# snphbaum/scikit-gpuppy

Measured on NVIDIA B200. Metric: fit_s_per_iter, lower is better.
Workload: dtype f64

## Files before the change

### scikit-gpuppy_b200/csrc/gpk.cu

```cuda
#include "../../include/gpk.h"
#include "../../include/gpk_test.h"

#include <climits>
#include <new>
#include <vector>

#include "dgemm_dmma.cuh"
#include "factor.cuh"
#include "se_kernels.cuh"
#include "exact_kernels.cuh"
#include "periodic_kernels.cuh"

namespace gpk {
thread_local char g_err[512] = {0};
thread_local long g_launch_count = 0;
thread_local bool g_prof_on = false;
static thread_local std::vector<ProfPair> g_prof;
void prof_push(cudaEvent_t a, cudaEvent_t b) { g_prof.push_back(ProfPair{a, b}); }

struct Handle {
  int n = 0, d = 0, npad = 0;
  double *X = nullptr, *W = nullptr;
  bool own_X = false, own_W = false;
  double *x = nullptr, *xT = nullptr, *t = nullptr, *y = nullptr, *alpha = nullptr, *dL = nullptr;
// ... 1088 lines not shown
  op.sl = reinterpret_cast<int8_t*>(planes_out); op.sc = scales_out;
  op.rows = (int)rows; op.K = (int)K; op.S = moduli;
  unsigned long long* mx = nullptr;
  GPK_CUDA_OK(cudaMalloc((void**)&mx, (size_t)rows * sizeof(unsigned long long)));
  int rc = oz::slice_operand(src, ld, trans, lower, op, mx, st);
  cudaError_t e = cudaStreamSynchronize(st);
  cudaFree(mx);
  if (rc < 0) return rc;
  if (e != cudaSuccess) { snprintf(g_err, sizeof(g_err), "oz_residues: %s", cudaGetErrorString(e)); return -1; }
  return 0;
}

int gpk_test_oz_gemm(const double* A, int64_t lda, int transA, int lowerA, const double* B, int64_t ldb, int transB,
                     int lowerB, double* C, int64_t ldc, int64_t M, int64_t N, int64_t K, double alpha, double beta,
                     int krange, int lower_only, int moduli, int64_t panel_rows, int reps, float* ms_out, void* stream) {
  cudaStream_t st = reinterpret_cast<cudaStream_t>(stream);
  oz::Operand a, b;
  a.rows = (int)M; a.K = (int)K; a.S = moduli;
  b.rows = (int)N; b.K = (int)K; b.S = moduli;
  unsigned long long* mx = nullptr;
  cudaEvent_t e0 = nullptr, e1 = nullptr, e2 = nullptr;
  int rc = 0;
  auto cleanup = [&]() {
    cudaFree(a.sl); cudaFree(a.sc); cudaFree(b.sl); cudaFree(b.sc); cudaFree(mx); cudaFree(a.out);
    if (e0) cudaEventDestroy(e0);
    if (e1) cudaEventDestroy(e1);
    if (e2) cudaEventDestroy(e2);
  };
#define OZ_OK(expr)                                                                         \
  do {                                                                                      \
    cudaError_t _e = (expr);                                                                \
    if (_e != cudaSuccess) {                                                                \
      snprintf(g_err, sizeof(g_err), "oz_gemm: %s -> %s", #expr, cudaGetErrorString(_e));   \
      cleanup();                                                                            \
      return -1;                                                                            \
    }                                                                                       \
  } while (0)
  OZ_OK(cudaMalloc((void**)&a.sl, oz::Operand::slice_bytes(a.rows, a.K, a.S)));
  OZ_OK(cudaMalloc((void**)&b.sl, oz::Operand::slice_bytes(b.rows, b.K, b.S)));
  OZ_OK(cudaMalloc((void**)&a.sc, (size_t)M * sizeof(double)));
  OZ_OK(cudaMalloc((void**)&b.sc, (size_t)N * sizeof(double)));
  OZ_OK(cudaMalloc((void**)&mx, (size_t)(M > N ? M : N) * sizeof(unsigned long long)));
  {
    const long prow = panel_rows > 0 ? round_up_l((long)panel_rows, 256) : round_up_l((long)M, 256);
    size_t want_out = (size_t)a.S * prow * round_up_l((long)N, 256);
    if (want_out > ((size_t)16 << 30)) want_out = (size_t)16 << 30;
    OZ_OK(cudaMalloc((void**)&a.out, want_out));
    a.out_cap = want_out;
  }
  OZ_OK(cudaEventCreate(&e0));
  OZ_OK(cudaEventCreate(&e1));
  OZ_OK(cudaEventCreate(&e2));
  OZ_OK(cudaEventRecord(e0, st));
  rc = oz::slice_operand(A, lda, transA, lowerA, a, mx, st);
  if (rc == 0) rc = oz::slice_operand(B, ldb, transB, lowerB, b, mx, st);
  if (rc < 0) { cleanup(); return rc; }
  OZ_OK(cudaEventRecord(e1, st));
  if (reps < 1) reps = 1;
  for (int r = 0; r < reps && rc == 0; ++r) rc = oz::gemm_sliced(a, b, C, ldc, alpha, beta, krange, lower_only, st);
  if (rc < 0) { cleanup(); return rc; }
  OZ_OK(cudaEventRecord(e2, st));
  OZ_OK(cudaStreamSynchronize(st));
  if (ms_out) {
    OZ_OK(cudaEventElapsedTime(&ms_out[0], e0, e1));
    OZ_OK(cudaEventElapsedTime(&ms_out[1], e1, e2));
    ms_out[1] /= reps;
  }
#undef OZ_OK
  cleanup();
  return 0;
}

int gpk_test_tune(int group_m, int recon_cw) {
  if (group_m > 0) oz::g_group_m = group_m;
  if (recon_cw == 1 || recon_cw == 2 || recon_cw == 4) oz::g_recon_cw = recon_cw;
  return 0;
}

int gpk_test_position_lock(int on) {
  if (on >= 0 && on <= 2) oz::g_position_lock = on;
  return oz::g_position_lock;
}

int gpk_test_overlap(int on) {
  if (on == 0 || on == 1) g_overlap_T = on;
  return g_overlap_T;
}

int gpk_profile(int on) {
  g_prof_on = on != 0;
  return 0;
}

int gpk_profile_read(double* gemm_ms, int64_t* gemm_launches, int64_t* all_launches, double* max_gemm_ms) {
  double total = 0.0, longest = 0.0;
  for (auto& p : g_prof) {
    float ms = 0.f;
    cudaError_t e = cudaEventSynchronize(p.b);
    if (e == cudaSuccess) e = cudaEventElapsedTime(&ms, p.a, p.b);
    cudaEventDestroy(p.a);
    cudaEventDestroy(p.b);
    if (e != cudaSuccess) {
      snprintf(g_err, sizeof(g_err), "gpk_profile_read: %s", cudaGetErrorString(e));
      g_prof.clear();
      return -1;
    }
    total += ms;
    if (ms > longest) longest = ms;
  }
  if (max_gemm_ms) *max_gemm_ms = longest;
  if (gemm_ms) *gemm_ms = total;
  if (gemm_launches) *gemm_launches = (int64_t)g_prof.size();
  if (all_launches) *all_launches = (int64_t)g_launch_count;
  g_prof.clear();
  g_launch_count = 0;
  return 0;
}

int gpk_microbench_i8(int64_t iters, double seconds, double* out_host) {
  int nsm = 0, dev = 0;
  GPK_CUDA_OK(cudaGetDevice(&dev));
  GPK_CUDA_OK(cudaDeviceGetAttribute(&nsm, cudaDevAttrMultiProcessorCount, dev));
  const int smem = 2 * oz::TILE_BYTES + 1024 + 64;
  GPK_CUDA_OK(cudaFuncSetAttribute(mb_i8_kernel, cudaFuncAttributeMaxDynamicSharedMemorySize, smem));
  cudaLaunchConfig_t cfg;
  memset(&cfg, 0, sizeof(cfg));
  cudaLaunchAttribute attr[1];
  attr[0].id = cudaLaunchAttributeClusterDimension;
  attr[0].val.clusterDim.x = 2;
  attr[0].val.clusterDim.y = 1;
  attr[0].val.clusterDim.z = 1;
  const int pairs = nsm / 2;
  cfg.gridDim = dim3(2 * pairs);
  cfg.blockDim = dim3(128);
  cfg.dynamicSmemBytes = smem;
  cfg.stream = nullptr;
  cfg.attrs = attr;
  cfg.numAttrs = 1;
  cudaEvent_t e0, e1;
  GPK_CUDA_OK(cudaEventCreate(&e0));
  GPK_CUDA_OK(cudaEventCreate(&e1));
  const double ops_per_launch = (double)pairs * (double)iters * 4.0 * 256.0 * 256.0 * 32.0 * 2.0;
  long it = iters;
  double best = 0.0;
  for (int rep = 0; rep < 4; ++rep) {
    GPK_CUDA_OK(cudaEventRecord(e0));
    GPK_CUDA_OK(cudaLaunchKernelEx(&cfg, mb_i8_kernel, it));
    GPK_LAUNCH_OK();
    GPK_CUDA_OK(cudaEventRecord(e1));
    GPK_CUDA_OK(cudaEventSynchronize(e1));
    float ms = 0.f;
    GPK_CUDA_OK(cudaEventElapsedTime(&ms, e0, e1));
    const double tops = ops_per_launch / (ms * 1e-3) / 1e12;
    if (rep > 0 && tops > best) best = tops;
  }
  out_host[0] = best;
  out_host[1] = 0.0;
  if (seconds > 0.0) {
    const double per_launch_s = ops_per_launch / (best * 1e12);
    long launches = (long)(seconds / per_launch_s) + 1;
    GPK_CUDA_OK(cudaEventRecord(e0));
    for (long l = 0; l < launches; ++l) {
      GPK_CUDA_OK(cudaLaunchKernelEx(&cfg, mb_i8_kernel, it));
      GPK_LAUNCH_OK();
    }
    GPK_CUDA_OK(cudaEventRecord(e1));
// ... 36 lines not shown
```

### scikit-gpuppy_b200/csrc/oz_crt_planes.cuh

```cuda

struct PlaneArgs {
  uint8_t* res; long res_ld; long res_plane;
  int M, N, K;
  int row_tile0;
  int krange, lower_only, group_m;
  int widen, band_cols;
  int nmod;
  unsigned int* phase;
  int* spill;
  int m[CRT_MAX_MODULI]; uint32_t magic[CRT_MAX_MODULI]; uint32_t u[CRT_MAX_MODULI];
};

constexpr int RECON_GROUPS = (CRT_MAX_MODULI + 3) / 4;

struct ReconArgs {
  const uint8_t* res; long res_ld; long res_plane;
  double* C; long ldc;
  const double* scA; const double* scB;
  double alpha, beta;
  int M, N, K;
  int row0;
  long ncols_pad;
  int krange, lower_only;
  int nmod;
  double p_scaled;
  double* colsq; double* pairdot; long ldo;
  uint32_t wp[2 * RECON_GROUPS][6];
};

constexpr int SPILL_SLOTS = 256;
constexpr int Q_BN = 256;
constexpr int Q_STAGES = 7;
constexpr int Q_STAGE_BYTES = 2 * TILE_BYTES;
constexpr int Q_SMEM_BYTES = Q_STAGES * Q_STAGE_BYTES + 1024 + 256;

__host__ __device__ __forceinline__ void planes_krange(int krange, int K, int bi2, int bx2, int& kb0, int& kb1) {
  kb0 = 0;
  kb1 = K / BK;
  switch (krange) {
    case K_UPTO_BJ: kb1 = (kb1 < 2 * bx2 + 2) ? kb1 : 2 * bx2 + 2; break;
    case K_FROM_BJ: kb0 = (kb1 < 2 * bx2) ? kb1 : 2 * bx2; break;
    case K_UPTO_BI: kb1 = (kb1 < 2 * bi2 + 2) ? kb1 : 2 * bi2 + 2; break;
    case K_FROM_BI: kb0 = (kb1 < 2 * bi2) ? kb1 : 2 * bi2; break;
    default: break;
  }
}

__global__ void __launch_bounds__(THREADS, 1)
oz_crt_planes_kernel(const __grid_constant__ CUtensorMap tmA, const __grid_constant__ CUtensorMap tmB,
                     const __grid_constant__ PlaneArgs p) {
  extern __shared__ uint8_t oz_smem_raw[];
  const int warp = threadIdx.x >> 5, lane = threadIdx.x & 31;
  const uint32_t rank = cluster_ctarank();
  const int pp = (int)(rank & 1u);

  int bx = blockIdx.x >> 1, by = blockIdx.y;
  const int nx = gridDim.x >> 1, ny = (int)gridDim.y;
  int band_lo = 0, band_hi = 0;
  if (p.group_m > 0) {
    const int pid = by * nx + bx;
    if (!p.band_cols) {
      const int per_band = p.group_m * nx;
      const int band = pid / per_band;
      const int first = band * p.group_m;
      const int rows = min(ny - first, p.group_m);
      const int rem = pid - band * per_band;
      by = first + rem % rows;
      bx = rem / rows;
      band_lo = first + p.row_tile0;
      band_hi = first + rows - 1 + p.row_tile0;
    } else {
      const int per_band = p.group_m * ny;
      const int band = pid / per_band;
      const int first = band * p.group_m;
      const int cols = min(nx - first, p.group_m);
      const int rem = pid - band * per_band;
      bx = first + rem % cols;
      by = rem / cols;
      band_lo = first;
      band_hi = first + cols - 1;
    }
  }
  const int bi2 = by + p.row_tile0;
  const int bi = 2 * bi2 + pp;
  const int bjt = 2 * bx + pp;
  if (p.lower_only && 2 * bx > 2 * bi2 + 1) return;
  int kb0, kb1;
  planes_krange(p.krange, p.K, bi2, bx, kb0, kb1);
  if (kb1 <= kb0) return;
  if (p.widen) {
    const int kbt = p.K / BK;
    switch (p.krange) {
      case K_FROM_BI: case K_FROM_BJ: { const int u = min(kb0, 2 * band_lo); kb0 = max(u, kb0 - WIDEN_TILES); if (kb0 < 0) kb0 = 0; } break;
      case K_UPTO_BI: case K_UPTO_BJ: { const int u = max(kb1, min(kbt, 2 * band_hi + 2)); kb1 = min(u, kb1 + WIDEN_TILES); if (kb1 > kbt) kb1 = kbt; } break;
      default: break;
    }
  }
  const int nmod = p.nmod;

  const uint32_t raw = smem_u32(oz_smem_raw);
  uint8_t* smem = oz_smem_raw + ((1024u - (raw & 1023u)) & 1023u);
  uint64_t* bars = reinterpret_cast<uint64_t*>(smem + Q_STAGES * Q_STAGE_BYTES);
  uint64_t* full = bars;
  uint64_t* empty = bars + Q_STAGES;
  uint64_t* tmem_full = bars + 2 * Q_STAGES;
  uint64_t* tmem_empty = bars + 2 * Q_STAGES + 2;
  uint32_t* tmem_slot = reinterpret_cast<uint32_t*>(bars + 2 * Q_STAGES + 4);

  if (warp == 0 && lane == 0) {
    tma_prefetch_desc(&tmA);
    tma_prefetch_desc(&tmB);
  }
  if (warp == 1 && lane == 0) {
    for (int s = 0; s < Q_STAGES; ++s) {
      mbar_init(&full[s], 1);
      mbar_init(&empty[s], 1);
    }
    for (int b = 0; b < 2; ++b) {
      mbar_init(&tmem_full[b], 1);
      mbar_init(&tmem_empty[b], 2 * EPI_WARPS);
    }
    fence_barrier_init();
  }
  if (warp == 2) tmem_alloc_pair(tmem_slot, TMEM_COLS);
  uint32_t* phase_slot = tmem_slot + 1;
  if (rank == 0 && threadIdx.x == 0) *phase_slot = p.phase ? *reinterpret_cast<volatile unsigned int*>(p.phase) : 0u;
  tc_fence_before();
  cluster_sync_all();
  tc_fence_after();
  const uint32_t tmem_base = *tmem_slot;
  uint32_t phase0;
  asm volatile(
      "{\n\t.reg .b32 ra;\n\t"
      "mapa.shared::cluster.u32 ra, %1, 0;\n\t"
      "ld.shared::cluster.u32 %0, [ra];\n\t}\n"
      : "=r"(phase0)
      : "r"(smem_u32(phase_slot))
      : "memory");
  uint32_t smid;
  asm volatile("mov.u32 %0, %%smid;" : "=r"(smid));
  const int nk = kb1 - kb0;
  uint32_t mstep0 = phase0 >> 16;
  int k_start = kb0 + (int)(phase0 & 0xffffu);
  if (k_start >= kb1) { k_start = kb0; ++mstep0; }
  const bool split = k_start > kb0 && p.spill != nullptr;
  if (!split) k_start = kb0;
  const int i0 = (int)(mstep0 % (uint32_t)nmod);
  const int nseg = nmod + (split ? 1 : 0);
#define SEG_MOD(sx) ((sx) < nmod ? ((i0 + (sx)) >= nmod ? i0 + (sx) - nmod : i0 + (sx)) : i0)
#define SEG_BEG(sx) ((split && (sx) == 0) ? k_start : kb0)
#define SEG_END(sx) ((split && (sx) == nmod) ? k_start : kb1)

  if (warp == 0) {
    if (lane == 0) {
      int stage = 0;
      uint32_t phase = 0;
      for (int sg = 0; sg < nseg; ++sg) {
        const int i = SEG_MOD(sg);
        const int kbeg = SEG_BEG(sg), kend = SEG_END(sg);
        for (int kb = kbeg; kb < kend; ++kb) {
          if (rank == 0 && p.phase && sg < nmod && ((kb - kbeg) & 3) == 0)
            atomicMax(p.phase, ((mstep0 + (uint32_t)sg) << 16) | (uint32_t)(kb - kb0));
          mbar_wait(&empty[stage], phase ^ 1u);
          uint8_t* st = smem + stage * Q_STAGE_BYTES;
          if (pp == 0) mbar_expect_tx(&full[stage], 2u * (uint32_t)Q_STAGE_BYTES);
          tma_load_tile_pair(st, &tmA, &full[stage], 0, kb, bi, i);
          tma_load_tile_pair(st + TILE_BYTES, &tmB, &full[stage], 0, kb, bjt, i);
          if (++stage == Q_STAGES) { stage = 0; phase ^= 1u; }
        }
      }
    }
  } else if (warp == 1) {
    if (lane == 0 && pp == 0) {
      constexpr uint32_t idesc = umma_idesc_i8(2 * BM, Q_BN);
      int stage = 0;
      uint32_t phase = 0;
      for (int sg = 0; sg < nseg; ++sg) {
        const int buf = sg & 1;
        if (sg >= 2) {
          mbar_wait(&tmem_empty[buf], (uint32_t)((sg >> 1) - 1) & 1u);
          tc_fence_after();
        }
        const uint32_t acc = tmem_base + (uint32_t)(buf * Q_BN);
        const int kbeg = SEG_BEG(sg), kend = SEG_END(sg);
        for (int kb = kbeg; kb < kend; ++kb) {
          mbar_wait(&full[stage], phase);
          tc_fence_after();
          const uint32_t st = smem_u32(smem + stage * Q_STAGE_BYTES);
          const uint64_t ad = umma_desc_sw128(st);
          const uint64_t bd = umma_desc_sw128(st + TILE_BYTES);
#pragma unroll
          for (int k4 = 0; k4 < BK / 32; ++k4)
            umma_i8_pair(acc, ad + (uint64_t)(k4 * 2), bd + (uint64_t)(k4 * 2), idesc, (kb > kbeg) | (k4 > 0));
          umma_commit_pair(&empty[stage], 3);
          if (++stage == Q_STAGES) { stage = 0; phase ^= 1u; }
        }
        umma_commit_pair(&tmem_full[buf], 3);
      }
    }
  } else {
    const int quad = warp & 3, half = (warp - 2) >> 2;
    const int row = quad * 32 + lane;
    const uint32_t lane_addr = tmem_base + ((uint32_t)(quad * 32) << 16);
    const long lrow = (long)by * (2 * BM) + pp * BM + row;
    uint8_t* dst0 = p.res + lrow * p.res_ld + (long)bx * Q_BN + half * 128;
    int4* sp = split ? reinterpret_cast<int4*>(p.spill + ((size_t)(smid % SPILL_SLOTS) * BM + row) * Q_BN + half * 128) : nullptr;
    for (int sg = 0; sg < nseg; ++sg) {
      const int i = SEG_MOD(sg);
      const bool spill_out = split && sg == 0, add_in = split && sg == nmod;
      const int buf = sg & 1;
      if (lane == 0) mbar_wait(&tmem_full[buf], (uint32_t)(sg >> 1) & 1u);
      __syncwarp();
      tc_fence_after();
      const int m = p.m[i];
      const int magic = (int)p.magic[i];
      const uint32_t u = p.u[i];
      uint8_t* dst = dst0 + (long)i * p.res_plane;
#pragma unroll
      for (int c = 0; c < 4; ++c) {
        uint32_t R[2][16];
        const uint32_t ta = lane_addr + (uint32_t)(buf * Q_BN + half * 128 + c * 32);
        tmem_ld16(ta, R[0]);
        tmem_ld16(ta + 16u, R[1]);
        tmem_ld_wait();
        if (c == 3) {
          tc_fence_before();
          __syncwarp();
          if (lane == 0) mbar_arrive_cluster(&tmem_empty[buf], rank & ~1u);
        }
        if (spill_out) {
#pragma unroll
          for (int x = 0; x < 8; ++x) {
            const uint32_t* r4 = &R[x >> 2][(x & 3) * 4];
            sp[c * 8 + x] = make_int4((int)r4[0], (int)r4[1], (int)r4[2], (int)r4[3]);
          }
          continue;
        }
        if (add_in) {
#pragma unroll
          for (int x = 0; x < 8; ++x) {
            const int4 v = sp[c * 8 + x];
            uint32_t* r4 = &R[x >> 2][(x & 3) * 4];
            r4[0] += (uint32_t)v.x; r4[1] += (uint32_t)v.y; r4[2] += (uint32_t)v.z; r4[3] += (uint32_t)v.w;
          }
        }
        uint32_t pk[8];
#pragma unroll
        for (int x = 0; x < 32; ++x) {
          const int Rv = (int)R[x >> 4][x & 15];
          const int r = Rv - __mulhi(Rv, magic) * m + m;
          const uint32_t t = (uint32_t)r * u;
          uint32_t s = t - __umulhi(t, (uint32_t)magic) * (uint32_t)m;
          s = (s >= (uint32_t)m) ? s - (uint32_t)m : s;
          if ((x & 3) == 0) pk[x >> 2] = s;
          else pk[x >> 2] |= s << (8 * (x & 3));
        }
        uint4* o = reinterpret_cast<uint4*>(dst + c * 32);
        o[0] = make_uint4(pk[0], pk[1], pk[2], pk[3]);
        o[1] = make_uint4(pk[4], pk[5], pk[6], pk[7]);
      }
    }
  }
#undef SEG_MOD
#undef SEG_BEG
#undef SEG_END
  tc_fence_before();
  cluster_sync_all();
  if (warp == 2) tmem_dealloc_pair(tmem_base, TMEM_COLS);
}

__device__ __forceinline__ uint32_t dp2a_lo(uint32_t a, uint32_t b, uint32_t c) {
  uint32_t d;
  asm("dp2a.lo.u32.u32 %0, %1, %2, %3;" : "=r"(d) : "r"(a), "r"(b), "r"(c));
  return d;
}
__device__ __forceinline__ uint32_t dp2a_hi(uint32_t a, uint32_t b, uint32_t c) {
  uint32_t d;
  asm("dp2a.hi.u32.u32 %0, %1, %2, %3;" : "=r"(d) : "r"(a), "r"(b), "r"(c));
  return d;
}
// ... 103 lines not shown
```

### scikit-gpuppy_b200/csrc/oz_gemm.cuh

```cuda
#pragma once
#include <cuda.h>

#include "dgemm_dmma.cuh"
#include "oz_crt_tables.h"

namespace gpk {
namespace oz {

constexpr int BM = 128, BN = 128, BK = 128;
constexpr int TILE_BYTES = BM * BK;
constexpr int EPI_WARPS = 8;
constexpr int THREADS = 64 + EPI_WARPS * 32;
constexpr int TMEM_COLS = 512;

constexpr int OZ_EPI_STORE = 0;
constexpr int OZ_EPI_ROWSQ = 1;

__device__ __forceinline__ uint32_t smem_u32(const void* p) { return (uint32_t)__cvta_generic_to_shared(p); }

__device__ __forceinline__ void mbar_init(uint64_t* bar, uint32_t count) {
  asm volatile("mbarrier.init.shared::cta.b64 [%0], %1;" ::"r"(smem_u32(bar)), "r"(count) : "memory");
}
__device__ __forceinline__ void fence_barrier_init() {
  asm volatile("fence.mbarrier_init.release.cluster;" ::: "memory");
}
__device__ __forceinline__ void mbar_expect_tx(uint64_t* bar, uint32_t bytes) {
  asm volatile("mbarrier.arrive.expect_tx.shared::cta.b64 _, [%0], %1;" ::"r"(smem_u32(bar)), "r"(bytes) : "memory");
}
__device__ __forceinline__ void mbar_arrive(uint64_t* bar) {
  asm volatile("mbarrier.arrive.shared::cta.b64 _, [%0];" ::"r"(smem_u32(bar)) : "memory");
}
__device__ __forceinline__ bool mbar_try_wait(uint64_t* bar, uint32_t parity) {
  uint32_t ok;
  asm volatile(
      "{\n\t.reg .pred p;\n\t"
      "mbarrier.try_wait.parity.shared::cta.b64 p, [%1], %2;\n\t"
      "selp.u32 %0, 1, 0, p;\n\t}\n"
      : "=r"(ok)
      : "r"(smem_u32(bar)), "r"(parity)
      : "memory");
  return ok != 0;
}
__device__ __forceinline__ void mbar_wait(uint64_t* bar, uint32_t parity) {
  if (mbar_try_wait(bar, parity)) return;
  const long long t0 = clock64();
  while (!mbar_try_wait(bar, parity)) {
    if (clock64() - t0 > 4000000000LL) __trap();
  }
}
__device__ __forceinline__ void tma_prefetch_desc(const CUtensorMap* tm) {
  asm volatile("prefetch.tensormap [%0];" ::"l"(tm) : "memory");
}
__device__ __forceinline__ void tc_fence_before() { asm volatile("tcgen05.fence::before_thread_sync;" ::: "memory"); }
__device__ __forceinline__ void tc_fence_after() { asm volatile("tcgen05.fence::after_thread_sync;" ::: "memory"); }
__device__ __forceinline__ void tmem_ld16(uint32_t taddr, uint32_t (&v)[16]) {
  asm volatile(
      "tcgen05.ld.sync.aligned.32x32b.x16.b32 {%0, %1, %2, %3, %4, %5, %6, %7, %8, %9, %10, %11, %12, %13, %14, %15}, "
      "[%16];"
      : "=r"(v[0]), "=r"(v[1]), "=r"(v[2]), "=r"(v[3]), "=r"(v[4]), "=r"(v[5]), "=r"(v[6]), "=r"(v[7]), "=r"(v[8]),
        "=r"(v[9]), "=r"(v[10]), "=r"(v[11]), "=r"(v[12]), "=r"(v[13]), "=r"(v[14]), "=r"(v[15])
      : "r"(taddr)
      : "memory");
}
__device__ __forceinline__ void tmem_ld_wait() { asm volatile("tcgen05.wait::ld.sync.aligned;" ::: "memory"); }

__device__ __forceinline__ uint32_t cluster_ctarank() {
  uint32_t r;
  asm volatile("mov.u32 %0, %%cluster_ctarank;" : "=r"(r));
  return r;
}
__device__ __forceinline__ void cluster_sync_all() {
  asm volatile("barrier.cluster.arrive.release.aligned;\n\tbarrier.cluster.wait.acquire.aligned;" ::: "memory");
}
__device__ __forceinline__ void mbar_arrive_cluster(uint64_t* bar, uint32_t rank) {
  asm volatile(
      "{\n\t.reg .b32 ra;\n\t"
      "mapa.shared::cluster.u32 ra, %0, %1;\n\t"
      "mbarrier.arrive.shared::cluster.b64 _, [ra];\n\t}\n"
      ::"r"(smem_u32(bar)), "r"(rank)
      : "memory");
}
__device__ __forceinline__ void tma_load_tile_pair(void* dst, const CUtensorMap* tm, uint64_t* bar, int row_in_tile,
                                                   int kb, int row_tile, int plane) {
  asm volatile(
      "cp.async.bulk.tensor.5d.cta_group::2.shared::cluster.global.mbarrier::complete_tx::bytes [%0], [%1, {%3, %4, %5, %6, "
      "%7}], [%2];"
      ::"r"(smem_u32(dst)), "l"(tm), "r"(smem_u32(bar) & 0xFEFFFFFFu), "r"(0), "r"(row_in_tile), "r"(kb), "r"(row_tile),
        "r"(plane)
      : "memory");
}
__device__ __forceinline__ void tmem_alloc_pair(uint32_t* dst_smem, uint32_t ncols) {
  asm volatile("tcgen05.alloc.cta_group::2.sync.aligned.shared::cta.b32 [%0], %1;" ::"r"(smem_u32(dst_smem)), "r"(ncols)
               : "memory");
  asm volatile("tcgen05.relinquish_alloc_permit.cta_group::2.sync.aligned;" ::: "memory");
}
__device__ __forceinline__ void tmem_dealloc_pair(uint32_t taddr, uint32_t ncols) {
  asm volatile("tcgen05.dealloc.cta_group::2.sync.aligned.b32 %0, %1;" ::"r"(taddr), "r"(ncols) : "memory");
}
__device__ __forceinline__ void umma_commit_pair(uint64_t* bar, uint16_t mask = 3) {
  asm volatile(
      "tcgen05.commit.cta_group::2.mbarrier::arrive::one.shared::cluster.multicast::cluster.b64 [%0], %1;"
      ::"r"(smem_u32(bar)), "h"(mask)
      : "memory");
}
__device__ __forceinline__ void umma_i8_pair(uint32_t tmem_d, uint64_t adesc, uint64_t bdesc, uint32_t idesc,
                                             uint32_t accumulate) {
  asm volatile(
      "{\n\t.reg .pred p;\n\t"
      "setp.ne.b32 p, %4, 0;\n\t"
      "tcgen05.mma.cta_group::2.kind::i8 [%0], %1, %2, %3, p;\n\t}\n"
      ::"r"(tmem_d), "l"(adesc), "l"(bdesc), "r"(idesc), "r"(accumulate)
      : "memory");
}
__device__ __forceinline__ double i32_to_f64(uint32_t v) {
  return __hiloint2double(0x43300000, (int)(v ^ 0x80000000u)) - 4503601774854144.0;
}

__device__ __forceinline__ uint64_t umma_desc_sw128(uint32_t smem_addr) {
  uint64_t d = 0;
  d |= (uint64_t)((smem_addr & 0x3FFFFu) >> 4);
  d |= (uint64_t)1 << 16;
  d |= (uint64_t)(1024 >> 4) << 32;
  d |= (uint64_t)1 << 46;
  d |= (uint64_t)2 << 61;
  return d;
}
__host__ __device__ constexpr uint32_t umma_idesc_i8(int M, int N) {
  return (2u << 4) | (1u << 7) | (1u << 10) | ((uint32_t)(N >> 3) << 17) | ((uint32_t)(M >> 4) << 24);
}

template <int TRANS>
__device__ __forceinline__ bool oz_valid(int r, int k, int lower) {
  if (!lower) return true;
  return TRANS ? ((r >> 7) <= (k >> 7)) : ((k >> 7) <= (r >> 7));
}
constexpr int WIDEN_MIN_K = 16384;
constexpr int WIDEN_TILES = 6;
inline int zero_fill_extra(int K) { return K >= WIDEN_MIN_K ? 1 + WIDEN_TILES : 1; }
template <int TRANS>
__device__ __forceinline__ bool oz_needed(int r, int k, int lower, int extra) {
  if (!lower) return true;
  return TRANS ? ((r >> 7) <= (k >> 7) + extra) : ((k >> 7) <= (r >> 7) + extra);
}

__device__ __forceinline__ size_t slice_offset(int rows, int K, int p, int r, int k) {
  const size_t tiles_per_plane = (size_t)(rows >> 7) * (size_t)(K >> 7);
  return (((size_t)p * tiles_per_plane + (size_t)(r >> 7) * (size_t)(K >> 7) + (size_t)(k >> 7)) << 14) +
         ((size_t)(r & 127) << 7) + (size_t)(k & 127);
}

__global__ void __launch_bounds__(256) oz_absmax_rows_kernel(const double* __restrict__ src, long ld, int K, int lower,
                                                             unsigned long long* __restrict__ mx) {
  __shared__ double red[8];
  const int r = blockIdx.x;
  const int kend = lower ? min(K, ((r >> 7) + 1) << 7) : K;
  const double* row = src + (long)r * ld;
  double m = 0.0;
  for (int k = threadIdx.x; k < kend; k += 256) m = fmax(m, fabs(row[k]));
#pragma unroll
  for (int o = 16; o > 0; o >>= 1) m = fmax(m, __shfl_xor_sync(0xffffffffu, m, o));
  if ((threadIdx.x & 31) == 0) red[threadIdx.x >> 5] = m;
  __syncthreads();
  if (threadIdx.x == 0) {
#pragma unroll
    for (int i = 0; i < 8; ++i) m = fmax(m, red[i]);
    mx[r] = (unsigned long long)__double_as_longlong(m);
  }
}
__global__ void __launch_bounds__(256) oz_absmax_cols_kernel(const double* __restrict__ src, long ld, int K, int lower,
                                                             unsigned long long* __restrict__ mx) {
  __shared__ double red[8][32];
// ... 122 lines not shown
  for (int i = 0; i < 16; ++i) oz_split(valid ? src[(long)(k0 + i) * ld + r] : 0.0, scale, lo[i], hi[i]);
  for (int p = 0; p < nmod; ++p)
    *reinterpret_cast<uint4*>(sl + slice_offset(rows, K, p, r, k0)) = oz_residues16(lo, hi, p);
}

#include "oz_crt_planes.cuh"

typedef CUresult (*EncodeTiledFn)(CUtensorMap*, CUtensorMapDataType, cuuint32_t, void*, const cuuint64_t*, const cuuint64_t*,
                                  const cuuint32_t*, const cuuint32_t*, CUtensorMapInterleave, CUtensorMapSwizzle,
                                  CUtensorMapL2promotion, CUtensorMapFloatOOBfill);

inline EncodeTiledFn encode_fn() {
  static EncodeTiledFn fn = [] {
    void* f = nullptr;
    cudaDriverEntryPointQueryResult q;
    if (cudaGetDriverEntryPoint("cuTensorMapEncodeTiled", &f, cudaEnableDefault, &q) != cudaSuccess ||
        q != cudaDriverEntryPointSuccess)
      f = nullptr;
    return reinterpret_cast<EncodeTiledFn>(f);
  }();
  return fn;
}

inline int make_tmap(CUtensorMap* tm, const int8_t* base, int rows, int K, int S, int box_rows = BM) {
  EncodeTiledFn enc = encode_fn();
  if (!enc) {
    snprintf(g_err, sizeof(g_err), "cuTensorMapEncodeTiled entry point not available");
    return -1;
  }
  const cuuint64_t kbs = (cuuint64_t)(K / BK), rts = (cuuint64_t)(rows / BM);
  cuuint64_t dims[5] = {(cuuint64_t)BK, (cuuint64_t)BM, kbs, rts, (cuuint64_t)S};
  cuuint64_t strides[4] = {(cuuint64_t)BK, (cuuint64_t)TILE_BYTES, (cuuint64_t)TILE_BYTES * kbs,
                           (cuuint64_t)TILE_BYTES * kbs * rts};
  cuuint32_t box[5] = {(cuuint32_t)BK, (cuuint32_t)box_rows, 1, 1, 1};
  cuuint32_t estr[5] = {1, 1, 1, 1, 1};
  CUresult r = enc(tm, CU_TENSOR_MAP_DATA_TYPE_UINT8, 5, const_cast<int8_t*>(base), dims, strides, box, estr,
                   CU_TENSOR_MAP_INTERLEAVE_NONE, CU_TENSOR_MAP_SWIZZLE_128B, CU_TENSOR_MAP_L2_PROMOTION_L2_256B,
                   CU_TENSOR_MAP_FLOAT_OOB_FILL_NONE);
  if (r != CUDA_SUCCESS) {
    snprintf(g_err, sizeof(g_err), "cuTensorMapEncodeTiled failed (%d) rows=%d K=%d S=%d", (int)r, rows, K, S);
    return -1;
  }
  return 0;
}
struct Operand {
  int8_t* sl = nullptr;
  double* sc = nullptr;
  int rows = 0, K = 0, S = 0;
  int bits = 0;
  uint8_t* out = nullptr;
  size_t out_cap = 0;
  static size_t slice_bytes(int rows, int K, int S) { return (size_t)S * rows * K; }
};

inline int slice_operand(const double* src, long ld, int trans, int lower, Operand& op, unsigned long long* mx,
                         cudaStream_t st) {
  if (op.rows % BM || op.K % BK || op.S < CRT_MIN_MODULI || op.S > CRT_MAX_MODULI) {
    snprintf(g_err, sizeof(g_err), "slice_operand: bad shape rows=%d K=%d moduli=%d", op.rows, op.K, op.S);
    return -2;
  }
  GPK_TRY(crt_upload_constants());
  op.bits = crt_bits(op.K, op.S);
  if (!trans) {
    oz_absmax_rows_kernel<<<op.rows, 256, 0, st>>>(src, ld, op.K, lower, mx);
    GPK_LAUNCH_OK();
    const long chunks = (long)op.rows * (op.K >> 4);
    oz_residue_rows_kernel<<<(unsigned)((chunks + 255) / 256), 256, 0, st>>>(src, ld, op.rows, op.K, lower, op.S,
                                                                            op.bits, zero_fill_extra(op.K), mx, op.sl, op.sc);
    GPK_LAUNCH_OK();
  } else {
    GPK_CUDA_OK(cudaMemsetAsync(mx, 0, (size_t)op.rows * sizeof(unsigned long long), st));
    dim3 g1(op.rows / 32, (op.K + 1023) / 1024);
    oz_absmax_cols_kernel<<<g1, 256, 0, st>>>(src, ld, op.K, lower, mx);
    GPK_LAUNCH_OK();
    dim3 g2(op.rows / 32, (op.K + 127) / 128);
    oz_residue_cols_kernel<<<g2, 256, 0, st>>>(src, ld, op.rows, op.K, lower, op.S, op.bits, zero_fill_extra(op.K), mx, op.sl, op.sc);
    GPK_LAUNCH_OK();
  }
  return 0;
}

thread_local int g_position_lock = 2;
thread_local int g_group_m = 4;
thread_local int g_recon_cw = 1;

inline int gemm_sliced(const Operand& A, const Operand& B, double* C, long ldc, double alpha, double beta, int krange,
                       int lower_only, cudaStream_t st, int epi = OZ_EPI_STORE, double* colsq = nullptr,
                       double* pairdot = nullptr, long ldo = 0) {
  if (A.K != B.K || A.S != B.S) {
    snprintf(g_err, sizeof(g_err), "gemm_sliced: operand mismatch K %d/%d moduli %d/%d", A.K, B.K, A.S, B.S);
    return -2;
  }
  if (A.bits != B.bits || A.bits != crt_bits(A.K, A.S)) {
    snprintf(g_err, sizeof(g_err), "gemm_sliced: operand widths %d/%d do not match K=%d", A.bits, B.bits, A.K);
    return -2;
  }
  const long Nc = ((long)B.rows + Q_BN - 1) / Q_BN * Q_BN;
  const size_t per_row = (size_t)A.S * (size_t)Nc;
  const long panel = (long)(A.out_cap / per_row) / 256 * 256;
  if (!A.out || panel < 256) {
    snprintf(g_err, sizeof(g_err), "gemm_sliced: the residue-plane buffer (%zu bytes) cannot hold a 256-row panel of %ld columns",
             A.out_cap, Nc);
    return -4;
  }
  static bool configured_on[GPK_MAX_DEVICES] = {};
  bool& configured = configured_on[current_device_slot()];
  if (!configured) {
    GPK_CUDA_OK(cudaFuncSetAttribute(oz_crt_planes_kernel, cudaFuncAttributeMaxDynamicSharedMemorySize, Q_SMEM_BYTES));
    configured = true;
  }
  CUtensorMap tmA, tmB;
  GPK_TRY(make_tmap(&tmA, A.sl, A.rows, A.K, A.S, BM));
  GPK_TRY(make_tmap(&tmB, B.sl, B.rows, B.K, B.S, BM));
  const CrtSet& cs = crt_set(A.S);
  PlaneArgs g;
  memset(&g, 0, sizeof(g));
  g.res = A.out; g.res_ld = Nc;
  g.M = A.rows; g.N = B.rows; g.K = A.K; g.krange = krange; g.lower_only = lower_only; g.nmod = A.S;
  g.group_m = g_group_m;
  g.widen = (g_position_lock >= 2 && g.group_m > 0 && g.group_m <= 4 && A.K >= WIDEN_MIN_K &&
             (krange == K_FROM_BI || krange == K_UPTO_BI || krange == K_FROM_BJ || krange == K_UPTO_BJ)) ? 1 : 0;
  g.band_cols = (g.widen && (krange == K_FROM_BJ || krange == K_UPTO_BJ)) ? 1 : 0;
  ReconArgs r;
  memset(&r, 0, sizeof(r));
  r.res = A.out; r.res_ld = Nc;
  r.C = C; r.ldc = ldc; r.scA = A.sc; r.scB = B.sc; r.alpha = alpha; r.beta = beta;
  r.M = A.rows; r.N = B.rows; r.K = A.K; r.krange = krange; r.lower_only = lower_only; r.nmod = A.S;
  r.p_scaled = cs.p_scaled;
  r.colsq = colsq; r.pairdot = pairdot; r.ldo = ldo;
  for (int i = 0; i < A.S; ++i) {
    g.m[i] = cs.mod[i].m; g.magic[i] = cs.mod[i].magic; g.u[i] = (uint32_t)cs.mod[i].u;
    const uint32_t w[3] = {cs.mod[i].w0, cs.mod[i].w1, cs.mod[i].w2};
    for (int j = 0; j < 6; ++j) {
      const uint32_t limb = (w[j >> 1] >> (16 * (j & 1))) & 0xffffu;
      r.wp[i >> 1][j] |= limb << (16 * (i & 1));
    }
  }
  static unsigned int* phase_dev_on[GPK_MAX_DEVICES] = {};
  unsigned int*& phase_dev = phase_dev_on[current_device_slot()];
  if (!phase_dev) GPK_CUDA_OK(cudaMalloc((void**)&phase_dev, 64 * sizeof(unsigned int)));
  static thread_local int phase_next = 0;
  static int* spill_dev_on[GPK_MAX_DEVICES] = {};
  int*& spill_dev = spill_dev_on[current_device_slot()];
  if (!spill_dev) GPK_CUDA_OK(cudaMalloc((void**)&spill_dev, (size_t)SPILL_SLOTS * BM * Q_BN * sizeof(int)));
  g.spill = g_position_lock ? spill_dev : nullptr;
  cudaEvent_t e0 = nullptr, e1 = nullptr;
  if (g_prof_on) {
    GPK_CUDA_OK(cudaEventCreate(&e0));
    GPK_CUDA_OK(cudaEventCreate(&e1));
    GPK_CUDA_OK(cudaEventRecord(e0, st));
  }
  for (long row0 = 0; row0 < A.rows; row0 += panel) {
    const long rows = (A.rows - row0 < panel) ? A.rows - row0 : panel;
    const long rows_pad = (rows + 255) / 256 * 256;
    g.row_tile0 = (int)(row0 / 256);
    g.res_plane = rows_pad * Nc;
    r.row0 = (int)row0;
    r.res_plane = g.res_plane;
    long ncol_tiles = Nc / Q_BN;
    if (lower_only && (row0 + rows_pad) / Q_BN < ncol_tiles) ncol_tiles = (row0 + rows_pad) / Q_BN;
    g.phase = phase_dev + (phase_next++ & 63);
    GPK_CUDA_OK(cudaMemsetAsync(g.phase, 0, sizeof(unsigned int), st));
    cudaLaunchConfig_t cfg;
    memset(&cfg, 0, sizeof(cfg));
    cudaLaunchAttribute attr[1];
    attr[0].id = cudaLaunchAttributeClusterDimension;
    attr[0].val.clusterDim.x = 2;
    attr[0].val.clusterDim.y = 1;
    attr[0].val.clusterDim.z = 1;
    cfg.gridDim = dim3((unsigned)(2 * ncol_tiles), (unsigned)(rows_pad / 256));
    cfg.blockDim = dim3(THREADS);
    cfg.dynamicSmemBytes = Q_SMEM_BYTES;
    cfg.stream = st;
    cfg.attrs = attr;
    cfg.numAttrs = 1;
    GPK_CUDA_OK(cudaLaunchKernelEx(&cfg, oz_crt_planes_kernel, tmA, tmB, g));
    GPK_LAUNCH_OK();
    long ncol_blocks = B.rows / 128;
    if (lower_only && (row0 + rows) / 128 < ncol_blocks) ncol_blocks = (row0 + rows) / 128;
    r.ncols_pad = ncol_blocks * 128;
    const int cw = g_recon_cw;
    dim3 rg((unsigned)((ncol_blocks + cw - 1) / cw), (unsigned)(rows / (8 / cw)));
    const int ng = (A.S + 3) / 4;
#define GPK_RECON2(NG, CW)                                                                           \
  do {                                                                                               \
    if (epi == OZ_EPI_STORE) oz_crt_reconstruct_kernel<OZ_EPI_STORE, NG, CW><<<rg, 256, 0, st>>>(r); \
    else oz_crt_reconstruct_kernel<OZ_EPI_ROWSQ, NG, CW><<<rg, 256, 0, st>>>(r);                     \
  } while (0)
#define GPK_RECON(NG)                       \
  do {                                      \
    if (cw == 1) GPK_RECON2(NG, 1);         \
    else if (cw == 2) GPK_RECON2(NG, 2);    \
    else GPK_RECON2(NG, 4);                 \
  } while (0)
    if (ng <= 2) GPK_RECON(2);
    else if (ng == 3) GPK_RECON(3);
    else if (ng == 4) GPK_RECON(4);
    else GPK_RECON(5);
#undef GPK_RECON
#undef GPK_RECON2
    GPK_LAUNCH_OK();
  }
  if (g_prof_on) {
    GPK_CUDA_OK(cudaEventRecord(e1, st));
    prof_push(e0, e1);
  }
  return 0;
}

struct Workspace {
  int8_t* buf = nullptr; size_t cap = 0, top = 0;
  double* sc = nullptr; size_t sc_cap = 0, sc_top = 0;
  unsigned long long* mx = nullptr; size_t mx_cap = 0;
  uint8_t* out = nullptr; size_t out_cap = 0;
  int S = CRT_MIN_MODULI;
  int min_dim = 2048;
  void reset() { top = 0; sc_top = 0; }
  Operand alloc(int rows, int K) {
    Operand op;
    const size_t bytes = Operand::slice_bytes(rows, K, S);
    if (top + bytes > cap || sc_top + (size_t)rows > sc_cap || (size_t)rows > mx_cap) return op;
    op.sl = buf + top; op.sc = sc + sc_top; op.rows = rows; op.K = K; op.S = S;
    op.out = out; op.out_cap = out_cap;
    top += bytes; sc_top += (size_t)rows;
    return op;
  }
  int ensure_out(size_t bytes) {
    if (bytes <= out_cap) return 0;
    if (out) cudaFree(out);
    out = nullptr; out_cap = 0;
    if (cudaMalloc((void**)&out, bytes) != cudaSuccess) { cudaGetLastError(); out = nullptr; return -1; }
    out_cap = bytes;
    return 0;
  }
  int ensure(size_t bytes, size_t rows_total, size_t rows_max) {
    if (bytes > cap) {
      if (buf) cudaFree(buf);
      buf = nullptr; cap = 0;
      if (cudaMalloc((void**)&buf, bytes) != cudaSuccess) { cudaGetLastError(); buf = nullptr; return -1; }
      cap = bytes;
    }
    if (rows_total > sc_cap) {
      if (sc) cudaFree(sc);
      sc = nullptr; sc_cap = 0;
      if (cudaMalloc((void**)&sc, rows_total * sizeof(double)) != cudaSuccess) { cudaGetLastError(); return -1; }
      sc_cap = rows_total;
    }
    if (rows_max > mx_cap) {
      if (mx) cudaFree(mx);
      mx = nullptr; mx_cap = 0;
      if (cudaMalloc((void**)&mx, rows_max * sizeof(unsigned long long)) != cudaSuccess) { cudaGetLastError(); return -1; }
      mx_cap = rows_max;
    }
    return 0;
  }
  void release() {
    if (buf) cudaFree(buf);
    if (sc) cudaFree(sc);
    if (mx) cudaFree(mx);
// ... 25 lines not shown
```

### scikit-gpuppy_b200/skgpuppy/_native.py

```python
import ctypes
import os

import numpy as np

_HERE = os.path.dirname(os.path.abspath(__file__))
_LIB_PATH = os.path.join(_HERE, "libgpk.so")
_lib = None

c_double_p = ctypes.POINTER(ctypes.c_double)
c_int_p = ctypes.POINTER(ctypes.c_int)
i64 = ctypes.c_int64
vp = ctypes.c_void_p

SIGNATURES = {
    "gpk_version": (ctypes.c_int, []),
    "gpk_last_error": (ctypes.c_char_p, []),
    "gpk_npad": (i64, [i64]),
    "gpk_create": (ctypes.c_int, [i64, i64, vp, vp, ctypes.POINTER(vp)]),
    "gpk_destroy": (ctypes.c_int, [vp]),
    "gpk_set_stream": (ctypes.c_int, [vp, vp]),
    "gpk_set_data": (ctypes.c_int, [vp, vp, vp]),
    "gpk_kernel_matrix": (ctypes.c_int, [vp, i64, vp, i64, i64, c_double_p, ctypes.c_int, vp, i64, vp]),
    "gpk_factorize": (ctypes.c_int, [vp, c_double_p, ctypes.c_int]),
    "gpk_factorize_matrix": (ctypes.c_int, [vp, vp, i64, ctypes.c_int]),
    "gpk_nll_matrix": (ctypes.c_int, [vp, c_double_p]),
    "gpk_logdet": (ctypes.c_int, [vp, c_double_p]),
    "gpk_nll_grad": (ctypes.c_int, [vp, c_double_p, c_double_p, c_double_p, ctypes.c_int]),
    "gpk_grad_trace_partial": (ctypes.c_int, [vp, i64, i64, c_double_p]),
    "gpk_solve": (ctypes.c_int, [vp, vp, i64, vp]),
    "gpk_inverse": (ctypes.c_int, [vp, vp, i64]),
    "gpk_solve_residual": (ctypes.c_int, [vp, c_double_p]),
    "gpk_get_alpha": (ctypes.c_int, [vp, vp]),
    "gpk_import_state": (ctypes.c_int, [vp, c_double_p, vp, ctypes.c_int]),
    "gpk_predict": (ctypes.c_int, [vp, vp, i64, ctypes.c_double, vp, vp, ctypes.c_int]),
    "gpk_predict_cross": (ctypes.c_int, [vp, vp, i64, i64, vp, ctypes.c_double, vp, vp]),
    "gpk_propagate_ga": (ctypes.c_int, [vp, vp, vp, i64, ctypes.c_int, ctypes.c_double, vp, vp]),
    "gpk_propagate_ga_parts": (ctypes.c_int, [vp, vp, vp, i64, ctypes.c_int, vp, vp]),
    "gpk_propagate_exact": (ctypes.c_int, [vp, vp, vp, vp, vp, i64, ctypes.c_double, vp, vp]),
    "gpk_set_kernel": (ctypes.c_int, [vp, ctypes.c_int]),
    "gpk_kernel_matrix_periodic": (ctypes.c_int, [vp, i64, vp, i64, i64, c_double_p, ctypes.c_int, vp, i64, vp]),
    "gpk_set_route": (ctypes.c_int, [vp, ctypes.c_int, i64, ctypes.c_int, i64]),
    "gpk_get_route": (ctypes.c_int, [vp, c_int_p]),
    "gpk_set_batch_rows": (ctypes.c_int, [vp, i64]),
}

TEST_SIGNATURES = {
    "gpk_test_gemm": (ctypes.c_int, [ctypes.c_int, ctypes.c_int, ctypes.c_int, vp, i64, vp, i64, vp, i64, i64, i64,
                                     i64, ctypes.c_double, ctypes.c_double, ctypes.c_int, ctypes.c_int, vp, vp, i64,
                                     vp]),
    "gpk_test_potrf_inv": (ctypes.c_int, [vp, vp, i64, i64, vp, c_int_p, vp]),
    "gpk_test_lauum": (ctypes.c_int, [vp, vp, i64, i64, vp]),
    "gpk_test_oz_residues": (ctypes.c_int, [vp, i64, i64, i64, ctypes.c_int, ctypes.c_int, ctypes.c_int, vp, vp, vp]),
    "gpk_test_oz_gemm": (ctypes.c_int, [vp, i64, ctypes.c_int, ctypes.c_int, vp, i64, ctypes.c_int, ctypes.c_int, vp, i64,
                                        i64, i64, i64, ctypes.c_double, ctypes.c_double, ctypes.c_int, ctypes.c_int,
                                        ctypes.c_int, i64, ctypes.c_int, ctypes.POINTER(ctypes.c_float), vp]),
    "gpk_test_tune": (ctypes.c_int, [ctypes.c_int, ctypes.c_int]),
    "gpk_test_overlap": (ctypes.c_int, [ctypes.c_int]),
    "gpk_test_position_lock": (ctypes.c_int, [ctypes.c_int]),
    "gpk_profile": (ctypes.c_int, [ctypes.c_int]),
    "gpk_profile_read": (ctypes.c_int, [c_double_p, ctypes.POINTER(i64), ctypes.POINTER(i64), c_double_p]),
    "gpk_microbench": (ctypes.c_int, [ctypes.c_int, i64, c_double_p]),
    "gpk_microbench_i8": (ctypes.c_int, [i64, ctypes.c_double, c_double_p]),
}


class GpkError(RuntimeError):
    pass


def lib_path():
    return _LIB_PATH


def load():
    global _lib
    if _lib is not None:
        return _lib
    if not os.path.exists(_LIB_PATH):
        raise GpkError(
            "libgpk.so not found at %s: build it with `python scikit-gpuppy_b200/build_native.py` "
            "(there is no CPU fallback)" % _LIB_PATH)
    lib = ctypes.CDLL(_LIB_PATH)
    for name, (res, args) in list(SIGNATURES.items()) + list(TEST_SIGNATURES.items()):
        fn = getattr(lib, name)
        fn.restype = res
        fn.argtypes = args
    _lib = lib
    return lib


def last_error():
    return load().gpk_last_error().decode("utf-8", "replace")


def check(rc, what=""):
    if rc == 0:
        return
    if rc > 0:
        raise np.linalg.LinAlgError("%s: leading minor %d of K is not positive definite" % (what, rc))
    raise GpkError("%s failed (%d): %s" % (what, rc, last_error()))


def theta_ptr(theta):
    th = np.ascontiguousarray(np.asarray(theta, dtype=np.float64))
    return th, th.ctypes.data_as(c_double_p)


def require_cuda():
    import torch
    if not torch.cuda.is_available():
        raise GpkError("no CUDA device: the skgpuppy B200 path has no CPU fallback")
    return torch


def ptr(t):
    if t is None:
        return None
    assert t.is_cuda and t.dtype.is_floating_point and t.element_size() == 8 and t.is_contiguous()
    return ctypes.c_void_p(t.data_ptr())


def current_stream_ptr():
    import torch
    return ctypes.c_void_p(torch.cuda.current_stream().cuda_stream)
```

Measured before the change: 0.3032.

## Multicast shared A/B tiles across larger clusters in CRT plane GEMM

Groups CTA pairs into 2x2 (or 1x2/2x1) clusters and uses TMA multicast so pairs that share a row or column tile load half-tiles once and broadcast them across the cluster. Tile mapping is recomputed from a linear grid with a preferred-cluster-dimension attribute, and empty barriers count arrivals from peer pairs. This is meant to reduce L2/global traffic for operand loads in the int8 Ozaki GEMM. In exchange it adds cross-pair synchronization, a drain loop at the end, and a fallback to non-shared loads when pairs have mismatched k-ranges.

```diff
diff --git a/scikit-gpuppy_b200/csrc/gpk.cu b/scikit-gpuppy_b200/csrc/gpk.cu
--- a/scikit-gpuppy_b200/csrc/gpk.cu
+++ b/scikit-gpuppy_b200/csrc/gpk.cu
@@ -1194,6 +1194,11 @@
   return oz::g_position_lock;
 }
 
+int gpk_test_cluster(int mode) {
+  if (mode >= 0 && mode <= 2) oz::g_cluster = mode;
+  return oz::g_cluster;
+}
+
 int gpk_test_overlap(int on) {
   if (on == 0 || on == 1) g_overlap_T = on;
   return g_overlap_T;
diff --git a/scikit-gpuppy_b200/csrc/oz_crt_planes.cuh b/scikit-gpuppy_b200/csrc/oz_crt_planes.cuh
--- a/scikit-gpuppy_b200/csrc/oz_crt_planes.cuh
+++ b/scikit-gpuppy_b200/csrc/oz_crt_planes.cuh
@@ -6,6 +6,8 @@
   int krange, lower_only, group_m;
   int widen, band_cols;
   int nmod;
+  int nx, ny;
+  int cm, cn;
   unsigned int* phase;
   int* spill;
   int m[CRT_MAX_MODULI]; uint32_t magic[CRT_MAX_MODULI]; uint32_t u[CRT_MAX_MODULI];
@@ -46,56 +48,104 @@
   }
 }
 
+struct PlaneTile {
+  int bx, by;
+  int kb0, kb1;
+  bool live;
+};
+__host__ __device__ inline PlaneTile planes_tile(const PlaneArgs& p, int pair) {
+  const int c = p.cm * p.cn;
+  const int cl = pair / c, q = pair - cl * c;
+  const int sx = (p.nx + p.cn - 1) / p.cn, sy = (p.ny + p.cm - 1) / p.cm;
+  int sbx = cl % sx, sby = cl / sx;
+  int band_lo = 0, band_hi = 0;
+  if (p.group_m > 0) {
+    if (!p.band_cols) {
+      const int gs = p.group_m / p.cm > 1 ? p.group_m / p.cm : 1;
+      const int per_band = gs * sx;
+      const int band = cl / per_band;
+      const int first = band * gs;
+      const int rows = (sy - first < gs) ? sy - first : gs;
+      const int rem = cl - band * per_band;
+      sby = first + rem % rows;
+      sbx = rem / rows;
+      band_lo = first * p.cm + p.row_tile0;
+      band_hi = ((first + rows) * p.cm < p.ny ? (first + rows) * p.cm : p.ny) - 1 + p.row_tile0;
+    } else {
+      const int gs = p.group_m / p.cn > 1 ? p.group_m / p.cn : 1;
+      const int per_band = gs * sy;
+      const int band = cl / per_band;
+      const int first = band * gs;
+      const int cols = (sx - first < gs) ? sx - first : gs;
+      const int rem = cl - band * per_band;
+      sbx = first + rem % cols;
+      sby = rem / cols;
+      band_lo = first * p.cn;
+      band_hi = ((first + cols) * p.cn < p.nx ? (first + cols) * p.cn : p.nx) - 1;
+    }
+  }
+  PlaneTile t;
+  t.by = sby * p.cm + q / p.cn;
+  t.bx = sbx * p.cn + q % p.cn;
+  const int bi2 = t.by + p.row_tile0;
+  planes_krange(p.krange, p.K, bi2, t.bx, t.kb0, t.kb1);
+  if (p.widen) {
+    const int kbt = p.K / BK;
+    switch (p.krange) {
+      case K_FROM_BI: case K_FROM_BJ: {
+        const int u = t.kb0 < 2 * band_lo ? t.kb0 : 2 * band_lo;
+        t.kb0 = u > t.kb0 - WIDEN_TILES ? u : t.kb0 - WIDEN_TILES;
+        if (t.kb0 < 0) t.kb0 = 0;
+      } break;
+      case K_UPTO_BI: case K_UPTO_BJ: {
+        const int hi = kbt < 2 * band_hi + 2 ? kbt : 2 * band_hi + 2;
+        const int u = t.kb1 > hi ? t.kb1 : hi;
+        t.kb1 = u < t.kb1 + WIDEN_TILES ? u : t.kb1 + WIDEN_TILES;
+        if (t.kb1 > kbt) t.kb1 = kbt;
+      } break;
+      default: break;
+    }
+  }
+  t.live = t.by < p.ny && t.bx < p.nx && !(p.lower_only && 2 * t.bx > 2 * bi2 + 1)
+           && t.kb1 > t.kb0;
+  return t;
+}
+
 __global__ void __launch_bounds__(THREADS, 1)
 oz_crt_planes_kernel(const __grid_constant__ CUtensorMap tmA, const __grid_constant__ CUtensorMap tmB,
+                     const __grid_constant__ CUtensorMap tmAh, const __grid_constant__ CUtensorMap tmBh,
                      const __grid_constant__ PlaneArgs p) {
   extern __shared__ uint8_t oz_smem_raw[];
   const int warp = threadIdx.x >> 5, lane = threadIdx.x & 31;
   const uint32_t rank = cluster_ctarank();
   const int pp = (int)(rank & 1u);
 
-  int bx = blockIdx.x >> 1, by = blockIdx.y;
-  const int nx = gridDim.x >> 1, ny = (int)gridDim.y;
-  int band_lo = 0, band_hi = 0;
-  if (p.group_m > 0) {
-    const int pid = by * nx + bx;
-    if (!p.band_cols) {
-      const int per_band = p.group_m * nx;
-      const int band = pid / per_band;
-      const int first = band * p.group_m;
-      const int rows = min(ny - first, p.group_m);
-      const int rem = pid - band * per_band;
-      by = first + rem % rows;
-      bx = rem / rows;
-      band_lo = first + p.row_tile0;
-      band_hi = first + rows - 1 + p.row_tile0;
-    } else {
-      const int per_band = p.group_m * ny;
-      const int band = pid / per_band;
-      const int first = band * p.group_m;
-      const int cols = min(nx - first, p.group_m);
-      const int rem = pid - band * per_band;
-      bx = first + rem % cols;
-      by = rem / cols;
-      band_lo = first;
-      band_hi = first + cols - 1;
-    }
-  }
+  const int npairs = p.cm * p.cn;
+  const int pair = (int)(blockIdx.x >> 1);
+  const int q = pair % npairs, qm = q / p.cn, qn = q % p.cn;
+  const PlaneTile tile = planes_tile(p, pair);
+  bool shared = npairs > 1 && (int)cluster_nctarank() == 2 * npairs;
+  for (int o = pair - q; shared && o < pair - q + npairs; ++o) {
+    const PlaneTile t = planes_tile(p, o);
+    shared = t.live && t.kb0 == tile.kb0 && t.kb1 == tile.kb1;
+  }
+  const int bx = tile.bx, by = tile.by, kb0 = tile.kb0, kb1 = tile.kb1;
+  const bool live = tile.live;
   const int bi2 = by + p.row_tile0;
   const int bi = 2 * bi2 + pp;
   const int bjt = 2 * bx + pp;
-  if (p.lower_only && 2 * bx > 2 * bi2 + 1) return;
-  int kb0, kb1;
-  planes_krange(p.krange, p.K, bi2, bx, kb0, kb1);
-  if (kb1 <= kb0) return;
-  if (p.widen) {
-    const int kbt = p.K / BK;
-    switch (p.krange) {
-      case K_FROM_BI: case K_FROM_BJ: { const int u = min(kb0, 2 * band_lo); kb0 = max(u, kb0 - WIDEN_TILES); if (kb0 < 0) kb0 = 0; } break;
-      case K_UPTO_BI: case K_UPTO_BJ: { const int u = max(kb1, min(kbt, 2 * band_hi + 2)); kb1 = min(u, kb1 + WIDEN_TILES); if (kb1 > kbt) kb1 = kbt; } break;
-      default: break;
-    }
-  }
+  const bool shareA = shared && p.cn > 1, shareB = shared && p.cm > 1;
+  const uint16_t own_pair = (uint16_t)(3u << (rank & ~1u));
+  uint16_t mcA = 0, mcB = 0, pairs_in = own_pair;
+  for (int j = 0; shareA && j < p.cn; ++j) {
+    mcA |= (uint16_t)(1u << (2 * (qm * p.cn + j) + pp));
+    pairs_in |= (uint16_t)(3u << (2 * (qm * p.cn + j)));
+  }
+  for (int i = 0; shareB && i < p.cm; ++i) {
+    mcB |= (uint16_t)(1u << (2 * (i * p.cn + qn) + pp));
+    pairs_in |= (uint16_t)(3u << (2 * (i * p.cn + qn)));
+  }
+  const uint32_t empty_count = 1u + (shareA ? 1u : 0u) + (shareB ? 1u : 0u);
   const int nmod = p.nmod;
 
   const uint32_t raw = smem_u32(oz_smem_raw);
@@ -110,11 +160,13 @@
   if (warp == 0 && lane == 0) {
     tma_prefetch_desc(&tmA);
     tma_prefetch_desc(&tmB);
+    if (shareA) tma_prefetch_desc(&tmAh);
+    if (shareB) tma_prefetch_desc(&tmBh);
   }
   if (warp == 1 && lane == 0) {
     for (int s = 0; s < Q_STAGES; ++s) {
       mbar_init(&full[s], 1);
-      mbar_init(&empty[s], 1);
+      mbar_init(&empty[s], empty_count);
     }
     for (int b = 0; b < 2; ++b) {
       mbar_init(&tmem_full[b], 1);
@@ -146,7 +198,8 @@
   const bool split = k_start > kb0 && p.spill != nullptr;
   if (!split) k_start = kb0;
   const int i0 = (int)(mstep0 % (uint32_t)nmod);
-  const int nseg = nmod + (split ? 1 : 0);
+  const int nseg = live ? nmod + (split ? 1 : 0) : 0;
+  const bool publisher = shared ? rank == 0 : pp == 0;
 #define SEG_MOD(sx) ((sx) < nmod ? ((i0 + (sx)) >= nmod ? i0 + (sx) - nmod : i0 + (sx)) : i0)
 #define SEG_BEG(sx) ((split && (sx) == 0) ? k_start : kb0)
 #define SEG_END(sx) ((split && (sx) == nmod) ? k_start : kb1)
@@ -159,15 +212,21 @@
         const int i = SEG_MOD(sg);
         const int kbeg = SEG_BEG(sg), kend = SEG_END(sg);
         for (int kb = kbeg; kb < kend; ++kb) {
-          if (rank == 0 && p.phase && sg < nmod && ((kb - kbeg) & 3) == 0)
+          if (publisher && p.phase && sg < nmod && ((kb - kbeg) & 3) == 0)
             atomicMax(p.phase, ((mstep0 + (uint32_t)sg) << 16) | (uint32_t)(kb - kb0));
           mbar_wait(&empty[stage], phase ^ 1u);
           uint8_t* st = smem + stage * Q_STAGE_BYTES;
           if (pp == 0) mbar_expect_tx(&full[stage], 2u * (uint32_t)Q_STAGE_BYTES);
-          tma_load_tile_pair(st, &tmA, &full[stage], 0, kb, bi, i);
-          tma_load_tile_pair(st + TILE_BYTES, &tmB, &full[stage], 0, kb, bjt, i);
+          if (shareA) tma_load_tile_pair_mc(st + qn * (TILE_BYTES / 2), &tmAh, &full[stage], qn * (BM / 2), kb, bi, i, mcA);
+          else tma_load_tile_pair(st, &tmA, &full[stage], 0, kb, bi, i);
+          if (shareB) tma_load_tile_pair_mc(st + TILE_BYTES + qm * (TILE_BYTES / 2), &tmBh, &full[stage], qm * (BM / 2), kb, bjt, i, mcB);
+          else tma_load_tile_pair(st + TILE_BYTES, &tmB, &full[stage], 0, kb, bjt, i);
           if (++stage == Q_STAGES) { stage = 0; phase ^= 1u; }
         }
+      }
+      for (int s = 0; s < Q_STAGES; ++s) {
+        mbar_wait(&empty[stage], phase ^ 1u);
+        if (++stage == Q_STAGES) { stage = 0; phase ^= 1u; }
       }
     }
   } else if (warp == 1) {
@@ -192,10 +251,10 @@
 #pragma unroll
           for (int k4 = 0; k4 < BK / 32; ++k4)
             umma_i8_pair(acc, ad + (uint64_t)(k4 * 2), bd + (uint64_t)(k4 * 2), idesc, (kb > kbeg) | (k4 > 0));
-          umma_commit_pair(&empty[stage], 3);
+          umma_commit_pair(&empty[stage], pairs_in);
           if (++stage == Q_STAGES) { stage = 0; phase ^= 1u; }
         }
-        umma_commit_pair(&tmem_full[buf], 3);
+        umma_commit_pair(&tmem_full[buf], own_pair);
       }
     }
   } else {
diff --git a/scikit-gpuppy_b200/csrc/oz_gemm.cuh b/scikit-gpuppy_b200/csrc/oz_gemm.cuh
--- a/scikit-gpuppy_b200/csrc/oz_gemm.cuh
+++ b/scikit-gpuppy_b200/csrc/oz_gemm.cuh
@@ -69,6 +69,11 @@
   asm volatile("mov.u32 %0, %%cluster_ctarank;" : "=r"(r));
   return r;
 }
+__device__ __forceinline__ uint32_t cluster_nctarank() {
+  uint32_t r;
+  asm volatile("mov.u32 %0, %%cluster_nctarank;" : "=r"(r));
+  return r;
+}
 __device__ __forceinline__ void cluster_sync_all() {
   asm volatile("barrier.cluster.arrive.release.aligned;\n\tbarrier.cluster.wait.acquire.aligned;" ::: "memory");
 }
@@ -87,6 +92,15 @@
       "%7}], [%2];"
       ::"r"(smem_u32(dst)), "l"(tm), "r"(smem_u32(bar) & 0xFEFFFFFFu), "r"(0), "r"(row_in_tile), "r"(kb), "r"(row_tile),
         "r"(plane)
+      : "memory");
+}
+__device__ __forceinline__ void tma_load_tile_pair_mc(void* dst, const CUtensorMap* tm, uint64_t* bar, int row_in_tile,
+                                                      int kb, int row_tile, int plane, uint16_t cta_mask) {
+  asm volatile(
+      "cp.async.bulk.tensor.5d.cta_group::2.shared::cluster.global.mbarrier::complete_tx::bytes.multicast::cluster [%0], [%1, "
+      "{%4, %5, %6, %7, %8}], [%2], %3;"
+      ::"r"(smem_u32(dst)), "l"(tm), "r"(smem_u32(bar) & 0xFEFFFFFFu), "h"(cta_mask), "r"(0), "r"(row_in_tile), "r"(kb),
+        "r"(row_tile), "r"(plane)
       : "memory");
 }
 __device__ __forceinline__ void tmem_alloc_pair(uint32_t* dst_smem, uint32_t ncols) {
@@ -375,6 +389,7 @@
 
 thread_local int g_position_lock = 2;
 thread_local int g_group_m = 4;
+thread_local int g_cluster = 2;
 thread_local int g_recon_cw = 1;
 
 inline int gemm_sliced(const Operand& A, const Operand& B, double* C, long ldc, double alpha, double beta, int krange,
@@ -405,6 +420,9 @@
   CUtensorMap tmA, tmB;
   GPK_TRY(make_tmap(&tmA, A.sl, A.rows, A.K, A.S, BM));
   GPK_TRY(make_tmap(&tmB, B.sl, B.rows, B.K, B.S, BM));
+  CUtensorMap tmAh, tmBh;
+  GPK_TRY(make_tmap(&tmAh, A.sl, A.rows, A.K, A.S, BM / 2));
+  GPK_TRY(make_tmap(&tmBh, B.sl, B.rows, B.K, B.S, BM / 2));
   const CrtSet& cs = crt_set(A.S);
   PlaneArgs g;
   memset(&g, 0, sizeof(g));
@@ -414,6 +432,13 @@
   g.widen = (g_position_lock >= 2 && g.group_m > 0 && g.group_m <= 4 && A.K >= WIDEN_MIN_K &&
              (krange == K_FROM_BI || krange == K_UPTO_BI || krange == K_FROM_BJ || krange == K_UPTO_BJ)) ? 1 : 0;
   g.band_cols = (g.widen && (krange == K_FROM_BJ || krange == K_UPTO_BJ)) ? 1 : 0;
+  g.cm = 1; g.cn = 1;
+  if (g_cluster == 1) {
+    if (krange == K_FROM_BJ || krange == K_UPTO_BJ) g.cm = 2;
+    else g.cn = 2;
+  } else if (g_cluster == 2 && A.K >= WIDEN_MIN_K && (g.widen || krange == K_FULL)) {
+    g.cm = g.cn = 2;
+  }
   ReconArgs r;
   memset(&r, 0, sizeof(r));
   r.res = A.out; r.res_ld = Nc;
@@ -456,18 +481,26 @@
     GPK_CUDA_OK(cudaMemsetAsync(g.phase, 0, sizeof(unsigned int), st));
     cudaLaunchConfig_t cfg;
     memset(&cfg, 0, sizeof(cfg));
-    cudaLaunchAttribute attr[1];
+    g.nx = (int)ncol_tiles;
+    g.ny = (int)(rows_pad / 256);
+    const long nclusters = (long)((g.nx + g.cn - 1) / g.cn) * ((g.ny + g.cm - 1) / g.cm);
+    const int cluster_ctas = 2 * g.cm * g.cn;
+    cudaLaunchAttribute attr[2];
     attr[0].id = cudaLaunchAttributeClusterDimension;
     attr[0].val.clusterDim.x = 2;
     attr[0].val.clusterDim.y = 1;
     attr[0].val.clusterDim.z = 1;
-    cfg.gridDim = dim3((unsigned)(2 * ncol_tiles), (unsigned)(rows_pad / 256));
+    attr[1].id = cudaLaunchAttributePreferredClusterDimension;
+    attr[1].val.preferredClusterDim.x = (unsigned)cluster_ctas;
+    attr[1].val.preferredClusterDim.y = 1;
+    attr[1].val.preferredClusterDim.z = 1;
+    cfg.gridDim = dim3((unsigned)(cluster_ctas * nclusters));
     cfg.blockDim = dim3(THREADS);
     cfg.dynamicSmemBytes = Q_SMEM_BYTES;
     cfg.stream = st;
     cfg.attrs = attr;
-    cfg.numAttrs = 1;
-    GPK_CUDA_OK(cudaLaunchKernelEx(&cfg, oz_crt_planes_kernel, tmA, tmB, g));
+    cfg.numAttrs = cluster_ctas > 2 ? 2 : 1;
+    GPK_CUDA_OK(cudaLaunchKernelEx(&cfg, oz_crt_planes_kernel, tmA, tmB, tmAh, tmBh, g));
     GPK_LAUNCH_OK();
     long ncol_blocks = B.rows / 128;
     if (lower_only && (row0 + rows) / 128 < ncol_blocks) ncol_blocks = (row0 + rows) / 128;
diff --git a/scikit-gpuppy_b200/skgpuppy/_native.py b/scikit-gpuppy_b200/skgpuppy/_native.py
--- a/scikit-gpuppy_b200/skgpuppy/_native.py
+++ b/scikit-gpuppy_b200/skgpuppy/_native.py
@@ -57,6 +57,7 @@
     "gpk_test_tune": (ctypes.c_int, [ctypes.c_int, ctypes.c_int]),
     "gpk_test_overlap": (ctypes.c_int, [ctypes.c_int]),
     "gpk_test_position_lock": (ctypes.c_int, [ctypes.c_int]),
+    "gpk_test_cluster": (ctypes.c_int, [ctypes.c_int]),
     "gpk_profile": (ctypes.c_int, [ctypes.c_int]),
     "gpk_profile_read": (ctypes.c_int, [c_double_p, ctypes.POINTER(i64), ctypes.POINTER(i64), c_double_p]),
     "gpk_microbench": (ctypes.c_int, [ctypes.c_int, i64, c_double_p]),
```

Result: faster. 0.2980, median of 6 (-1.7%).
